# VinAIResearch/LFM

Measured on AMD Instinct MI355X. Metric: images/sec, higher is better.
Workload: dtype f16; 1 GPU; DiT-L/2 celeb256 f8 (4x32x32 latents), batch 64/GPU, 50-step Euler (torchdiffeq grid) + f8 VAE decode to 256x256 + uint8 NHWC; 2 batches in flight on 2 HIP streams (same weights, own scratch); per_gpu_batch=64, global_batch=64, h2d_of_latents=inside the timed step, nfe=50, batches_in_flight=2

## Files before the change

### include/lfm_hip.h

```cpp
#ifndef LFM_HIP_H
#define LFM_HIP_H
#include <stddef.h>
#include <stdint.h>

#ifdef __cplusplus
extern "C" {
#endif

typedef void* lfm_stream_t;

#define LFM_OK 0
#define LFM_ERR_SHAPE (-1)
#define LFM_ERR_ALIGN (-2)
#define LFM_ERR_WORKSPACE (-3)
#define LFM_ERR_LAUNCH (-4)
#define LFM_ERR_ARG (-5)

const char* lfm_strerror(int code);
#define LFM_ABI_VERSION 4
int lfm_abi_version(void);

typedef struct lfm_dit_shape {
  int depth;
  int hidden;
// ... 47 lines not shown
  int fold_ln;
  int gemm_select;
} lfm_dit_call;
#define LFM_CALL_OFF 1
#define LFM_CALL_ON 2
#define LFM_CALL_GEMM_SELECT(which) ((which) + 1)

size_t lfm_dit_workspace_bytes(const lfm_dit_shape* shape, int max_batch);

int lfm_dit_forward(const lfm_dit_shape* shape, const lfm_dit_weights* w, void* workspace, size_t workspace_bytes,
                    const lfm_dit_call* call, lfm_stream_t stream);

#define LFM_PLAN_FOLDED_LN 1
#define LFM_PLAN_FUSED_QKV_ATTENTION 2
int lfm_dit_plan(const lfm_dit_shape* shape, const lfm_dit_call* call, int* plan_out);

size_t lfm_dit_cond_table_bytes(const lfm_dit_shape* shape, int n_times);
int lfm_dit_cond_table_build(const lfm_dit_shape* shape, const lfm_dit_weights* w, void* workspace, size_t workspace_bytes, int batch, const float* t_values,
                             int n_times, void* table, size_t table_bytes, lfm_stream_t stream);

int lfm_gemm_f16(const void* A, long lda, const void* W, long ldw, void* C, long ldc, int M, int N, int K, const float* bias,
                 int epilogue, const float* gate, long gate_stride, int tokens, lfm_stream_t stream);

int lfm_gemm_qkv_f16(const void* A, long lda, const void* W, long ldw, void* Q, void* K_out, void* Vt, int M, int D, int K,
                     const float* bias, int head_dim, int tokens, lfm_stream_t stream);

int lfm_gemm_select(int which);
int lfm_gemm_plan(int M, int N, int K, int batch, int caps);

int lfm_profile_fc1(int enable);
int lfm_profile_blocks_read(float* host_ms_out, int max_n);
#define LFM_OPT_FOLD_LN 1
#define LFM_OPT_GEMM_V6 2
#define LFM_OPT_SKINNY_GEMM 4
#define LFM_OPT_ATTENTION_STREAM 5
#define LFM_OPT_FUSED_QKV_ATTENTION 6
int lfm_set_option(int key, int value);
int lfm_dit_call_settings(const lfm_dit_call* call, int* gemm_select_out, int* fold_ln_out);

int lfm_clock_probe(int blocks, int iters, unsigned long long* ticks_out, lfm_stream_t stream);

#ifdef LFM_MEASURE
int lfm_gemm_trace_read(unsigned long long* host_out, int n_per_group);
int lfm_attention_trace_read(unsigned long long* host_out, int n);
int lfm_attention_wg_trace_read(unsigned long long* host_out, int n_wg);
int lfm_dit_chk_arm(const void* workspace);
int lfm_dit_chk_read(unsigned long long* host_out, int n);
#endif
int lfm_profile_fc1_read(float* host_ms_out, int max_n);

int lfm_ln_modulate(const float* X, void* A, int M, int D, int tokens, const float* shift, const float* scale, long mod_stride,
// ... 95 lines not shown
```

### lfm_amd/csrc/dit.hip

```cpp
#include <mutex>

#include "../../include/lfm_hip.h"
#include "gemm_dispatch.h"
#include "gemm_skinny_kernel.h"
#include "gemm_sq64_kernel.h"
#include "qkv_attention_kernel.h"

typedef std::atomic<int> Opt;
static inline int opt_get(const Opt& o) { return o.load(std::memory_order_relaxed); }
static inline void opt_set(Opt& o, int v) { o.store(v, std::memory_order_relaxed); }
static struct {
  Opt gemm_sel{0}, gemm_dbg{0};
  Opt fold_ln{1};
  Opt v6{0};
  Opt skinny{1};
  Opt stagger{0};
  Opt att_stream{1};
  Opt fused_qkv{1};
} g_def;
static thread_local int tl_sel_set = 0, tl_gemm_sel = 0, tl_gemm_dbg = 0;
static thread_local int tl_fold = 0;
static inline int gemm_sel() { return tl_sel_set ? tl_gemm_sel : opt_get(g_def.gemm_sel); }
static inline int gemm_dbg() { return tl_sel_set ? tl_gemm_dbg : opt_get(g_def.gemm_dbg); }
static inline int opt_fold_ln() { return tl_fold ? (tl_fold == LFM_CALL_ON ? 1 : 0) : opt_get(g_def.fold_ln); }
int lfm_gemm_selected() { return gemm_sel(); }
int lfm_gemm_debug_flags() { return gemm_dbg(); }
int lfm_gemm_selected_v1_ok() { return gemm_sel() < 2 && !(gemm_dbg() & LFM_DBG_GEMM_NO_SPLITK); }
int lfm_gemm_prefers_v4(int M, int N, int K) {
  (void)M;
  (void)N;
  (void)K;
  if (gemm_dbg() & LFM_DBG_GEMM_NEVER_V4) return 0;
  if (gemm_dbg() & LFM_DBG_GEMM_ALWAYS_V4) return 1;
// ... 46 lines not shown
  }
  if (key == 2) {
    opt_set(g_def.v6, value != 0);
    return LFM_OK;
  }
  if (key == 4) {
    opt_set(g_def.skinny, value < 0 || value > 2 ? 1 : value);
    return LFM_OK;
  }
  if (key == 5) {
    opt_set(g_def.att_stream, value != 0);
    return LFM_OK;
  }
  if (key == 6) {
    opt_set(g_def.fused_qkv, value != 0);
    return LFM_OK;
  }
#ifdef LFM_MEASURE
  if (key == 3) {
    opt_set(g_def.stagger, value > 0 ? value : 0);
    return LFM_OK;
  }
#endif
  return LFM_ERR_ARG;
}
extern "C" int lfm_gemm_select(int which) {
  if (!gemm_select_valid(which)) return LFM_ERR_ARG;
  opt_set(g_def.gemm_sel, which & 15);
  opt_set(g_def.gemm_dbg, which >> 4);
  return LFM_OK;
// ... 1104 lines not shown
  const DitWs ws = carve(s, batch, workspace);
  if (ws.total > workspace_bytes) return LFM_ERR_WORKSPACE;
  if (((uintptr_t)workspace & 255) || ((uintptr_t)table & 15)) return LFM_ERR_ALIGN;
  hipStream_t st = (hipStream_t)stream;
  for (int i = 0; i < n_times; ++i) {
    rc = dit_conditioning(s, w, ws, t_values + i, 1, nullptr, 1, cond_uv_shape(s), st);
    if (rc) return rc;
    rc = dit_cond_copy(s, ws, (const float*)table, nullptr, 0, i, 1, st, n_times);
    if (rc) return rc;
  }
  return LFM_OK;
}

struct DitPlan {
  bool fold, w6, fused;
};
static DitPlan dit_plan(const lfm_dit_shape* s, int B, int rows) {
  const int D = s->hidden, H = s->mlp_hidden, grid = s->res / s->patch, T = grid * grid, M = B * T;
  const int tiles_p = D / 256;
  DitPlan p;
  p.fold = opt_fold_ln() && (D % 256 == 0) && (M % 256 == 0) && (rows == 1 || T % 256 == 0) && (long)(M / 256) * tiles_p >= 192 &&
           (gemm_sel() == 0 || gemm_sel() == 6) && (H % 64 == 0) && s->depth >= 1;
  p.w6 = gemm_sel() == 6 || (gemm_sel() == 0 && opt_get(g_def.v6));
  p.fused = p.fold && opt_get(g_def.fused_qkv) && !p.w6 && T == 256 && D == s->heads * 64 && (long)M * D < (1L << 31) && (long)3 * D * D < (1L << 31);
  return p;
}
extern "C" int lfm_dit_plan(const lfm_dit_shape* s, const lfm_dit_call* c, int* plan_out) {
  int rc = check_shape(s);
  if (rc) return rc;
  if (!c || !plan_out) return LFM_ERR_ARG;
  const int B = c->batch;
  if (B <= 0 || (c->t_len != 1 && c->t_len != B)) return LFM_ERR_SHAPE;
  CallScope scope;
  if ((rc = call_scope_enter(c)) != LFM_OK) return rc;
  const DitPlan p = dit_plan(s, B, (c->t_len == 1 && !c->y) ? 1 : B);
  *plan_out = (p.fold ? LFM_PLAN_FOLDED_LN : 0) | (p.fused ? LFM_PLAN_FUSED_QKV_ATTENTION : 0);
  return LFM_OK;
}

extern "C" int lfm_dit_forward(const lfm_dit_shape* s, const lfm_dit_weights* w, void* workspace, size_t workspace_bytes,
                               const lfm_dit_call* c, lfm_stream_t stream) {
  int rc = check_shape(s);
  if (rc) return rc;
  if (!w || !workspace || !c || !c->x || !c->t || !c->out) return LFM_ERR_ARG;
  const int B = c->batch;
  if (B <= 0 || (c->t_len != 1 && c->t_len != B)) return LFM_ERR_SHAPE;
  const bool cfg = c->cfg != 0;
  if (cfg && (B & 1)) return LFM_ERR_SHAPE;
  if (c->axpy_base && !c->axpy_dt) return LFM_ERR_ARG;
  const DitWs ws = carve(s, B, workspace);
  if (ws.total > workspace_bytes) return LFM_ERR_WORKSPACE;
// ... 47 lines not shown
  int cen_cur = 0;
  if (fold) {
    if (!pe_mfma) {
      hipLaunchKernelGGL(ln_center_mod_kernel, dim3(cdiv(M, 4)), dim3(256), 0, st, ws.X, ws.A, M, D, T, ws.mod + D, mstride, ws.ln_part, tiles_p,
                         ws.cen[0]);
      LFM_CHECK_LAUNCH();
    }
  }
  auto rowstat_src = [&]() {
    RowStatSrc r{ws.ln_part, ws.cen[cen_cur], ws.cen[cen_cur ^ 1], tiles_p, 1.0f / (float)D, 1e-6f};
    cen_cur ^= 1;
    return r;
  };
  auto launch_fold = [&](const ASrcRowMajor& a, const half_t* Wp, long ldw_, int M_, int N_, int K_, const auto& e) {
    return w6 ? launch_gemm256w_tn(a, Wp, ldw_, M_, N_, K_, e, st) : launch_gemm256h_tn(a, Wp, ldw_, M_, N_, K_, e, st);
  };
#ifdef LFM_MEASURE
  const bool chk = g_chk && workspace == g_chk_ws;
  if (chk) (void)hipMemsetAsync(g_chk, 0, DIT_CHK_SLOTS * 8, st);
#define DIT_CHK(buf, bytes, slot) \
  if (chk) dit_chk(buf, bytes, i, slot, st)
#else
#define DIT_CHK(buf, bytes, slot)
#endif
  const bool prof_blk = prof_ok && g_prof_blk_count < LFM_PROF_BLK_MAX;
  if (prof_blk) (void)hipEventRecord(g_prof_blk_ev[2 * g_prof_blk_count], st);
  const bool fused = plan.fused;
  if (fold) {
    for (int i = 0; i < s->depth; ++i) {
      const float* mod = ws.mod + (long)i * 6 * D;
// ... 3 lines not shown
      half_t* A1b = fused ? ws.A : ws.A2;
      if (fused) {
        const QkvAttnArgs e_qa{uq, uq + (long)rows * 3 * D, uvs_q, rowstat_src(), Ob, D, s->heads, 0.125f * 1.4426950408889634f, nullptr, 0};
        rc = launch_qkv_attention(ws.A, D, (const half_t*)w->qkv_w + (size_t)i * 3 * D * D, D, M, D, s->heads, D, e_qa, st);
        if (rc) return rc;
      } else {
        const EpiQKVMod e_qkv{Qb, Kb, Vb, uq, uq + (long)rows * 3 * D, uvs_q, D, D / s->heads, T, EpiQKV::log2_or_neg(T), rowstat_src(), nullptr, 0};
        rc = launch_fold(ASrcRowMajor{ws.A, D, M, 0}, (const half_t*)w->qkv_w + (size_t)i * 3 * D * D, D, M, 3 * D, D, e_qkv);
        if (rc) return rc;
        DIT_CHK(ws.QKVH, (size_t)3 * M * D * 2, 0);
        rc = attention_launch(Qb, Kb, Vb, Ob, B, s->heads, D / s->heads, T, st);
        if (rc) return rc;
      }
      DIT_CHK(Ob, (size_t)M * D * 2, 1);
      const EpiGateResidMod e_proj{ws.X, D, w->proj_b + (size_t)i * D, mod + 2 * D, mstride, T, A1b, mod + 4 * D, mstride, ws.cen[cen_cur], ws.ln_part, tiles_p};
      rc = launch_fold(ASrcRowMajor{Ob, D, M, 0}, (const half_t*)w->proj_w + (size_t)i * D * D, D, M, D, D, e_proj);
      if (rc) return rc;
      DIT_CHK(ws.X, (size_t)M * D * 4, 2);
      DIT_CHK(A1b, (size_t)M * D * 2, 3);
      DIT_CHK(ws.ln_part, (size_t)M * tiles_p * 8, 4);
      const bool prof = prof_ok && g_prof_mode == 1 && g_prof_count < LFM_PROF_MAX;
      if (prof) (void)hipEventRecord(g_prof_ev[2 * g_prof_count], st);
#if defined(LFM_MEASURE) && defined(LFM_EXP_DUMP)
      const EpiModGeluF16 e_fc1{ws.QKVH, H, uf, uf + (long)rows * H, uvs_f, T, rowstat_src(), nullptr, 0,
                                (g_dbg && workspace == g_dbg_ws) ? g_dbg + (long)i * g_dbg_stride : (float*)nullptr};
#else
      const EpiModGeluF16 e_fc1{ws.QKVH, H, uf, uf + (long)rows * H, uvs_f, T, rowstat_src(), nullptr, 0};
#endif
      rc = launch_fold(ASrcRowMajor{A1b, D, M, 0}, (const half_t*)w->fc1_w + (size_t)i * H * D, D, M, H, D, e_fc1);
      if (rc) return rc;
      if (prof) (void)hipEventRecord(g_prof_ev[2 * g_prof_count++ + 1], st);
      DIT_CHK(ws.QKVH, (size_t)M * H * 2, 5);
      if (i + 1 < s->depth) {
        const EpiGateResidMod e_fc2{ws.X, D, w->fc2_b + (size_t)i * D, mod + 5 * D, mstride, T, ws.A, mod + 7 * D, mstride, ws.cen[cen_cur], ws.ln_part, tiles_p};
        rc = launch_fold(ASrcRowMajor{ws.QKVH, H, M, 0}, (const half_t*)w->fc2_w + (size_t)i * D * H, H, M, D, H, e_fc2);
      } else {
        const EpiGateResidF32 e_fc2{ws.X, D, w->fc2_b + (size_t)i * D, mod + 5 * D, mstride, T};
        rc = launch_fold(ASrcRowMajor{ws.QKVH, H, M, 0}, (const half_t*)w->fc2_w + (size_t)i * D * H, H, M, D, H, e_fc2);
      }
      if (rc) return rc;
      DIT_CHK(ws.X, (size_t)M * D * 4, 6);
      DIT_CHK(ws.A, (size_t)M * D * 2, 7);
    }
  }
#undef DIT_CHK
  auto sk_slices = [&](int N_, int K_) {
    int sl = 1;
    while ((N_ / SK_BN) * (sl * 2) <= 256 && (K_ % (sl * 2 * SK_BK)) == 0 && K_ / (sl * 2) >= 2 * SK_BK && (size_t)(sl * 2) * M * N_ * 4 <= ws.slab_bytes) sl *= 2;
    return sl;
  };
// ... 170 lines not shown
```

### lfm_amd/csrc/gemm256h_kernel.h

```cpp
#pragma once
#include "gemm256n_kernel.h"

typedef float f32x4_t __attribute__((ext_vector_type(4)));

template <bool TRACE>
__device__ __forceinline__ void g256h_stamp(bool tr, int g, int wn, int lane, int slot) {
  if constexpr (TRACE) {
    if (tr && wn == 0 && lane == 0) {
      unsigned long long t;
      asm volatile("s_memtime %0\n\ts_waitcnt lgkmcnt(0)" : "=s"(t)::"memory");
      g256q_trace[g][slot] = t;
    }
  }
}

template <class Epi, class = void>
struct epi_has_row_aux {
  static constexpr bool value = false;
};
template <class Epi>
struct epi_has_row_aux<Epi, decltype((void)&Epi::row_aux)> {
  static constexpr bool value = true;
};

// ... 125 lines not shown
      for (int ps = 0; ps < 8; ++ps)
        if (mb + ps * 4 < M) epi.store(mb + ps * 4, n, v[ps], epi.load(mb + ps * 4, n));
    }
    asm volatile("s_waitcnt lgkmcnt(0)" ::: "memory");
  }
}

__device__ __forceinline__ float g256h_row16_sum(float v) {
  v = dpp_add<0xB1>(v);
  v = dpp_add<0x4E>(v);
  v = dpp_add<0x124>(v);
  v = dpp_add<0x128>(v);
  return v;
}

template <class Epi>
__device__ __forceinline__ void g256h_epilogue_mod(f32x4_t (&acc)[8][4], char* smem, const Epi& epi, int m0, int n0, int tile_n, int N, int g, int wn,
                                                   int lane, int wave) {
  char* scr = smem + wave * (32 * 272);
  float* red = (float*)(smem + 8 * 32 * 272);
  float* cen_s = (float*)(smem + 8 * 32 * 272 + 8192);
  const int l15 = lane & 15, l4 = lane >> 4;
  const int rrow = lane >> 4, rcol = lane & 15;
  const int n = n0 + wn * 64 + rcol * 4;
  const int img = m0 / epi.tokens;
  if (threadIdx.x < 256) cen_s[threadIdx.x] = epi.cen[m0 + threadIdx.x];
  const f32x4 bias = *(const f32x4*)(epi.bias + n);
  const f32x4 gate = *(const f32x4*)(epi.gate + (long)img * epi.gate_stride + n);
  const f32x4 sc1 = *(const f32x4*)(epi.scale + (long)img * epi.mod_stride + n) + 1.0f;
  __syncthreads();
#pragma unroll
  for (int i = 0; i < 4; ++i) {
#pragma unroll
    for (int h2 = 0; h2 < 2; ++h2)
#pragma unroll
      for (int j = 0; j < 4; ++j) *(f32x4_t*)(scr + (h2 * 16 + l15) * 272 + (j * 16 + l4 * 4) * 4) = acc[2 * i + h2][j];
    asm volatile("s_waitcnt lgkmcnt(0)" ::: "memory");
    const int rl = g * 128 + i * 32 + rrow;
    f32x4 xo[8];
#pragma unroll
    for (int ps = 0; ps < 8; ++ps) xo[ps] = *(const f32x4*)(epi.X + (long)(m0 + rl + ps * 4) * epi.ldx + n);
#pragma unroll
    for (int ps = 0; ps < 8; ++ps) {
      const f32x4 v = *(const f32x4*)(scr + (ps * 4 + rrow) * 272 + rcol * 16);
      const float c = cen_s[rl + ps * 4];
      const f32x4 xn = xo[ps] + gate * (v + bias);
      *(f32x4*)(epi.X + (long)(m0 + rl + ps * 4) * epi.ldx + n) = xn;
      const f32x4 d = xn - c;
      const f32x4 ap = d * sc1;
      const half4_t h = {(half_t)ap.x, (half_t)ap.y, (half_t)ap.z, (half_t)ap.w};
      *(half4_t*)(epi.A + (long)(m0 + rl + ps * 4) * N + n) = h;
      const float sx = g256h_row16_sum((xn.x + xn.y) + (xn.z + xn.w));
      const float sq = g256h_row16_sum((d.x * d.x + d.y * d.y) + (d.z * d.z + d.w * d.w));
      if (rcol == 0) {
        float* dst = red + (((g * 4 + wn) * 128) + i * 32 + ps * 4 + rrow) * 2;
        dst[0] = sx;
// ... 6 lines not shown
  if (wn == 0) {
#pragma unroll
    for (int rr = 0; rr < 2; ++rr) {
      const int r = lane + 64 * rr;
      float sx = 0.f, sq = 0.f;
#pragma unroll
      for (int w4 = 0; w4 < 4; ++w4) {
        sx += red[((g * 4 + w4) * 128 + r) * 2];
        sq += red[((g * 4 + w4) * 128 + r) * 2 + 1];
      }
      *(f32x2*)(epi.part + ((long)(m0 + g * 128 + r) * epi.tiles_n + tile_n) * 2) = (f32x2){sx, sq};
    }
  }
}

#define G256H_MAX_PARTS 5
struct G256hRowStatRegs {
  f32x2 p[G256H_MAX_PARTS];
  float c;
};
template <class Epi>
__device__ __forceinline__ G256hRowStatRegs g256h_rowstat_load(const Epi& epi, int m0, int M) {
  G256hRowStatRegs r;
  const int m = m0 + (int)threadIdx.x < M ? m0 + (int)threadIdx.x : M - 1;
  if (threadIdx.x < 256) {
    const f32x2* pp = (const f32x2*)(epi.st.part + (long)m * epi.st.tiles_p * 2);
#pragma unroll
    for (int t = 0; t < G256H_MAX_PARTS; ++t) r.p[t] = t < epi.st.tiles_p ? pp[t] : (f32x2){0.f, 0.f};
    r.c = epi.st.cen_in[m];
  }
// ... 163 lines not shown

  typename ASrc::Row arow[2][2];
  const half_t* wrow[2][2];
  const int cswz = ((tid & 7) ^ ((tid >> 4) & 7)) * 8;
#pragma unroll
  for (int s = 0; s < 2; ++s)
#pragma unroll
    for (int p = 0; p < 2; ++p) {
      arow[s][p] = asrc.row(m0 + p * 128 + s * 64 + (tid >> 3));
      const int n = n0 + (p * 2 + (tid >> 8)) * 64 + s * 32 + ((tid >> 3) & 31);
      wrow[s][p] = W + (long)(n < N ? n : N - 1) * ldw + cswz;
    }
  const int nk = K / G256Q_BK;
  const int dma_off = wave * 1024;
  bool dma_on = true;
  constexpr bool BUFDMA = (OPT & 1) != 0 && asrc_has_buffer<ASrc>::value;
  __amdgpu_buffer_rsrc_t rsa, rsw;
  unsigned avoff[2][2], wvoff[2][2];
  if constexpr (BUFDMA) {
    rsa = asrc.rsrc();
    rsw = __builtin_amdgcn_make_buffer_rsrc((void*)W, 0, -1, 0x00020000);
#pragma unroll
    for (int s = 0; s < 2; ++s)
#pragma unroll
      for (int p = 0; p < 2; ++p) {
        avoff[s][p] = asrc.voff(arow[s][p], cswz);
        const int n = n0 + (p * 2 + (tid >> 8)) * 64 + s * 32 + ((tid >> 3) & 31);
        wvoff[s][p] = ((unsigned)(n < N ? n : N - 1) * (unsigned)ldw + (unsigned)cswz) * 2u;
      }
  }
// ... 59 lines not shown
        }
        return;
      }
      if constexpr (PH == 0) {
        if (s1) issue_b(1, t + 1, oth + G256Q_SLOT_B1, P);
      } else if constexpr (PH == 1) {
        if (s1) issue_a(1, oth + G256Q_SLOT_A1, P);
      } else if constexpr (PH == 2) {
        if (s2) {
          if (P != 2) asrc.begin_tile(t + 2, G256Q_BK);
          issue_a(0, cur + G256Q_SLOT_A0, P);
        }
      } else {
        if (s2) issue_b(0, t + 2, cur + G256Q_SLOT_B0, P);
      }
    };
    if constexpr ((OPT & 2) != 0) {
      stage(1);
      __builtin_amdgcn_sched_barrier(0);
    }
    if constexpr (PH == 0) {
#pragma unroll
      for (int ks = 0; ks < 2; ++ks) {
        lds_read(wf[0][ks], w_addr[ks] + HI, g256q_ic<G256Q_SLOT_B0>{});
        lds_read(wf[1][ks], w_addr[ks] + HI, g256q_ic<G256Q_SLOT_B0 + 2048>{});
        lds_read(af[0][ks], a_addr[ks] + HI, g256q_ic<G256Q_SLOT_A0>{});
        lds_read(af[1][ks], a_addr[ks] + HI, g256q_ic<G256Q_SLOT_A0 + 2048>{});
        lds_read(af[2][ks], a_addr[ks] + HI, g256q_ic<G256Q_SLOT_A0 + 4096>{});
        lds_read(af[3][ks], a_addr[ks] + HI, g256q_ic<G256Q_SLOT_A0 + 6144>{});
      }
// ... 2 lines not shown
      for (int ks = 0; ks < 2; ++ks) {
        lds_read(wf[2][ks], w_addr[ks] + HI, g256q_ic<G256Q_SLOT_B1>{});
        lds_read(wf[3][ks], w_addr[ks] + HI, g256q_ic<G256Q_SLOT_B1 + 2048>{});
      }
    } else if constexpr (PH == 2) {
#pragma unroll
      for (int ks = 0; ks < 2; ++ks) {
        lds_read(af[0][ks], a_addr[ks] + HI, g256q_ic<G256Q_SLOT_A1>{});
        lds_read(af[1][ks], a_addr[ks] + HI, g256q_ic<G256Q_SLOT_A1 + 2048>{});
        lds_read(af[2][ks], a_addr[ks] + HI, g256q_ic<G256Q_SLOT_A1 + 4096>{});
        lds_read(af[3][ks], a_addr[ks] + HI, g256q_ic<G256Q_SLOT_A1 + 6144>{});
      }
    }
    __builtin_amdgcn_sched_barrier(0);
    stage((OPT & 2) != 0 ? 2 : 0);
    if constexpr (ABL == 1 || ABL == 3 || (ABL >= 5 && ABL <= 7)) {
      G256H_VMCNT(0);
    } else if constexpr ((OPT & 4) != 0) {
      if (s1) {
        if constexpr (PH < 3) G256H_VMCNT(4);
        else if (s2) G256H_VMCNT(6);
        else G256H_VMCNT(2);
      } else G256H_VMCNT(0);
    } else if (s2) G256H_VMCNT(6);
    else if (s1) {
      if constexpr (PH < 2) G256H_VMCNT(6);
      else if constexpr (PH == 2) G256H_VMCNT(4);
      else G256H_VMCNT(2);
    } else G256H_VMCNT(0);
  };
  auto mfma_part = [&](auto PHC, auto SWC) {
// ... 42 lines not shown
            if constexpr (SW) asm volatile("v_mfma_f32_16x16x32_f16 %0, %1, %2, %0" : "+v"(acc[I0 + i4][J0 + j2]) : "v"(af[i4][ks]), "v"(wf[J0 + j2][ks]));
            else asm volatile("v_mfma_f32_16x16x32_f16 %0, %1, %2, %0" : "+v"(acc[I0 + i4][J0 + j2]) : "v"(wf[J0 + j2][ks]), "v"(af[i4][ks]));
          } else if constexpr (SW) acc[I0 + i4][J0 + j2] = __builtin_amdgcn_mfma_f32_16x16x32_f16(af[i4][ks], wf[J0 + j2][ks], acc[I0 + i4][J0 + j2], 0, 0, 0);
          else acc[I0 + i4][J0 + j2] = __builtin_amdgcn_mfma_f32_16x16x32_f16(wf[J0 + j2][ks], af[i4][ks], acc[I0 + i4][J0 + j2], 0, 0, 0);
        }
        __builtin_amdgcn_sched_barrier(0);
      }
    if constexpr (ABL != 4) __builtin_amdgcn_s_setprio(0);
  };

  G256hRowStatRegs rsr;
  if constexpr (epi_has_rowstat<Epi>::value) {
    rsr = g256h_rowstat_load(epi, m0, M);
    __builtin_amdgcn_sched_barrier(0);
  }
  asrc.begin_tile(0, G256Q_BK);
  issue_a(0, smem + G256Q_SLOT_A0);
  issue_b(0, 0, smem + G256Q_SLOT_B0);
  issue_b(1, 0, smem + G256Q_SLOT_B1);
  issue_a(1, smem + G256Q_SLOT_A1);
  if (nk > 1) {
    asrc.begin_tile(1, G256Q_BK);
    issue_a(0, smem + G256Q_BUF_BYTES + G256Q_SLOT_A0);
    issue_b(0, 1, smem + G256Q_BUF_BYTES + G256Q_SLOT_B0);
  }
  if constexpr (epi_has_rowstat<Epi>::value) g256h_rowstat_finish(epi, rsr, smem, m0, M, tile_n);
  if (nk > 1) G256H_VMCNT(6);
  else G256H_VMCNT(2);
  if constexpr (ABL == 1 || ABL == 3 || (ABL >= 5 && ABL <= 7)) {
    G256H_VMCNT(0);
    dma_on = false;
  }
  if constexpr (ABL == 2 || ABL == 3 || (ABL >= 5 && ABL <= 7)) {
#pragma unroll
    for (int i = 0; i < 4; ++i)
#pragma unroll
      for (int ks = 0; ks < 2; ++ks) {
        af[i][ks] = (half8_t){1, 2, 3, 4, 5, 6, 7, 8};
        wf[i][ks] = (half8_t){1, -1, 1, -1, 1, -1, 1, -1};
      }
  }
  if constexpr (ABL == 4) {
    if (g == 1) __builtin_amdgcn_s_setprio(1);
  }
  G256_BARRIER();
  auto run = [&](auto GC, auto SWC) {
    constexpr int G = decltype(GC)::value;
    if constexpr (G == 0) load_part(g256q_ic<0>{}, g256q_ic<0>{}, 0, 1 < nk, 2 < nk);
    G256_BARRIER();
    auto tile = [&](auto BUFC, int t) {
      constexpr int BUF = decltype(BUFC)::value;
      const bool s1 = t + 1 < nk, s2 = t + 2 < nk, s3 = t + 3 < nk;
      auto phase = [&](auto PHC) {
        constexpr int PH = decltype(PHC)::value;
        if constexpr (G == 0) {
          mfma_part(PHC, SWC);
          if constexpr (PH < 3) load_part(g256q_ic<PH + 1>{}, BUFC, t, s1, s2);
          else if (s1) load_part(g256q_ic<0>{}, g256q_ic<(BUF ^ 1)>{}, t + 1, s2, s3);
        } else {
          load_part(PHC, BUFC, t, s1, s2);
          mfma_part(PHC, SWC);
        }
        if constexpr (ABL == 5 || ABL == 7) {
        } else if constexpr (ABL == 6) {
// ... 17 lines not shown
  if constexpr (epi_has_transposed<Epi>::value) {
    if (swapped) {
      if (g == 0) run(g256q_ic<0>{}, g256q_ic<1>{});
      else run(g256q_ic<1>{}, g256q_ic<1>{});
    } else {
      if (g == 0) run(g256q_ic<0>{}, g256q_ic<0>{});
      else run(g256q_ic<1>{}, g256q_ic<0>{});
    }
  } else {
    if (g == 0) run(g256q_ic<0>{}, g256q_ic<0>{});
    else run(g256q_ic<1>{}, g256q_ic<0>{});
  }
#undef G256H_VMCNT
#undef G256H_LGKM
  if constexpr (ABL == 7 || ABL == 8) asm volatile("s_nop 7\n\ts_nop 7\n\ts_nop 7" ::: "memory");
  g256h_epilogue<G256_BN, TRACE>(acc, smem, epi, m0, n0, M, N, g, wn, lane, wave, bz, bsC, dbg, swapped);
}

template <class ASrc, class Epi, bool TRACE = false, int ABL = 0, int OPT = G256H_DEFAULT_OPT>
static inline int launch_gemm256h_tn(const ASrc& asrc, const half_t* W, long ldw, int M, int N, int K, const Epi& epi, hipStream_t stream,
                                     int batch = 1, long bsA = 0, long bsW = 0, long bsC = 0) {
  if (!asrc_fits(asrc, 0)) return LFM_ERR_SHAPE;
  if constexpr ((OPT & 1) != 0 && asrc_has_buffer<ASrc>::value) {
    if (!asrc_fits_buffer(asrc, 0) || (long)N * ldw >= (1L << 31)) return LFM_ERR_SHAPE;
  }
  if (M <= 0 || N <= 0 || K <= 0 || (K % G256Q_BK) != 0 || (N % 4) != 0) return LFM_ERR_SHAPE;
  if ((ldw % 8) != 0 || ((uintptr_t)W & 15)) return LFM_ERR_ALIGN;
  const int tm = cdiv(M, G256_BM), tn = cdiv(N, G256_BN);
  constexpr int LDS = G256Q_LDS_BYTES + (epi_has_rowstat<Epi>::value ? 2048 : 0);
  static lfm_device_mask attr_set{0};
  const unsigned long long dbit = lfm_device_bit();
  if (lfm_device_todo(attr_set, dbit)) {
    if (hipFuncSetAttribute((const void*)gemm256h_tn_kernel<ASrc, Epi, TRACE, ABL, OPT>, hipFuncAttributeMaxDynamicSharedMemorySize, LDS) != hipSuccess)
      return LFM_ERR_LAUNCH;
    lfm_device_done(attr_set, dbit);
  }
  hipLaunchKernelGGL((gemm256h_tn_kernel<ASrc, Epi, TRACE, ABL, OPT>), dim3(tm * tn, batch), dim3(512), LDS, stream, asrc, W, ldw, M, N, K, tn, epi, bsA,
                     bsW, bsC, lfm_gemm_debug_flags());
  LFM_CHECK_LAUNCH();
  return LFM_OK;
}
```

### lfm_amd/csrc/gemm_kernel.h

```cpp
#pragma once
#include "common.h"
#include "debug_flags.h"

#define GEMM_BM 128
#define GEMM_BN 128
#define GEMM_BK 64
#define GEMM_STAGE_BYTES (2 * GEMM_BM * GEMM_BK * 2)
#define GEMM_LDS_BYTES (2 * GEMM_STAGE_BYTES)

struct ASrcRowMajor {
  const half_t* A;
  long lda;
  int M;
  __device__ __forceinline__ void init(int bz, long bs) { A += (long)bz * bs; }
  struct Row {
    unsigned off;
  };
  __device__ __forceinline__ Row row(int m) const {
    Row r;
    r.off = (unsigned)((m < M ? m : M - 1) * (int)lda);
    return r;
  }
  int k0;
  __device__ __forceinline__ void begin_tile(int kt, int bk) { k0 = kt * bk; }
// ... 164 lines not shown
    a.x = *(const f32x4*)(X + (long)m * ldx + n);
    return a;
  }
  __device__ __forceinline__ void store(int m, int n, f32x4 v, const Aux& a) const {
    *(f32x4*)(X + (long)m * ldx + n) = a.x + a.g * (v + a.b);
  }
};
template <class Epi, class = void>
struct epi_is_producer_mod {
  static constexpr bool value = false;
};
template <class Epi>
struct epi_is_producer_mod<Epi, decltype((void)Epi::producer_mod)> {
  static constexpr bool value = Epi::producer_mod;
};

struct EpiModF16 {
  half_t* C;
  long ldc;
  const float* u;
  const float* v;
  long uv_stride;
  int tokens;
  const float* rs;
  int m0;
  struct Aux {
    f32x4 u, v;
  };
  static constexpr bool column_aux = true;
  __device__ __forceinline__ Aux load(int m, int n) const {
// ... 569 lines not shown
```

### lfm_amd/hip.py

```python
import ctypes as C
import os

import torch

_HERE = os.path.dirname(os.path.abspath(__file__))
LIB_PATH = os.path.join(_HERE, "_lib", "liblfm_hip.so")
_lib = None


class LfmHipError(RuntimeError):
    pass


class DitShape(C.Structure):
    _fields_ = [(n, C.c_int) for n in ("depth", "hidden", "heads", "patch", "in_ch", "res", "mlp_hidden", "label_rows")]


_DIT_WEIGHT_FIELDS = ("pos_embed", "patch_w", "patch_b", "t_w0", "t_b0", "t_w2", "t_b2", "y_table", "ada_w", "ada_b",
                      "qkv_w", "qkv_b", "proj_w", "proj_b", "fc1_w", "fc1_b", "fc2_w", "fc2_b", "final_w", "final_b", "patch_w16")


class DitWeights(C.Structure):
    _fields_ = [(n, C.c_void_p) for n in _DIT_WEIGHT_FIELDS]

# ... 69 lines not shown
    L.lfm_profile_fc1.argtypes = [C.c_int]
    L.lfm_profile_fc1_read.restype = C.c_int
    L.lfm_profile_fc1_read.argtypes = [C.POINTER(C.c_float), C.c_int]
    L.lfm_profile_blocks_read.restype = C.c_int
    L.lfm_profile_blocks_read.argtypes = [C.POINTER(C.c_float), C.c_int]
    L.lfm_ln_modulate.restype = C.c_int
    L.lfm_ln_modulate.argtypes = [C.c_void_p, C.c_void_p, C.c_int, C.c_int, C.c_int, C.c_void_p, C.c_void_p, C.c_long, C.c_void_p]
    L.lfm_dit_attention.restype = C.c_int
    L.lfm_dit_attention.argtypes = [C.c_void_p, C.c_void_p, C.c_void_p, C.c_void_p, C.c_int, C.c_int, C.c_int, C.c_void_p]
    L.lfm_set_option.restype = C.c_int
    L.lfm_set_option.argtypes = [C.c_int, C.c_int]
    L.lfm_dit_call_settings.restype = C.c_int
    L.lfm_dit_call_settings.argtypes = [C.POINTER(DitCall), C.POINTER(C.c_int), C.POINTER(C.c_int)]
    L.lfm_dit_plan.restype = C.c_int
    L.lfm_dit_plan.argtypes = [C.POINTER(DitShape), C.POINTER(DitCall), C.POINTER(C.c_int)]
    L.lfm_gemm_plan.restype = C.c_int
    L.lfm_gemm_plan.argtypes = [C.c_int] * 5
    L.lfm_dit_attention_hd.restype = C.c_int
    L.lfm_dit_attention_hd.argtypes = [C.c_void_p, C.c_void_p, C.c_void_p, C.c_void_p, C.c_int, C.c_int, C.c_int, C.c_int, C.c_void_p]
    L.lfm_grid_advance.restype = C.c_int
    L.lfm_grid_advance.argtypes = [C.c_void_p] * 7
    L.lfm_lincomb.restype = C.c_int
    L.lfm_lincomb.argtypes = [C.c_void_p, C.c_void_p, C.POINTER(C.c_void_p), C.c_void_p, C.c_void_p, C.c_int, C.c_long, C.c_void_p]
    L.lfm_rk_error_norm.restype = C.c_int
    L.lfm_rk_error_norm.argtypes = [C.c_void_p, C.c_void_p, C.POINTER(C.c_void_p), C.c_void_p, C.c_void_p, C.c_int, C.c_long, C.c_float, C.c_float,
                                    C.c_void_p, C.c_void_p, C.c_void_p]
    L.lfm_vae_workspace_bytes.restype = C.c_size_t
    L.lfm_vae_workspace_bytes.argtypes = [C.c_int, C.c_int]
    L.lfm_vae_decode.restype = C.c_int
    L.lfm_vae_decode.argtypes = [C.c_void_p, C.c_void_p, C.c_size_t, C.c_void_p, C.c_void_p, C.c_int, C.c_int, C.c_int, C.c_void_p]
# ... 149 lines not shown
DBG_LN_FOUR_ROWS = 262144
DBG_LN_TWO_ROWS = 524288
DBG_DIT_FINAL_ROUND1 = 1048576
DBG_DIT_PATCH_ROUND1 = 2097152
DBG_CONV_IMPLICIT_GEMM = 8388608
DBG_CONV_HALO_SMALL = 16777216
DBG_VAE_SEPARATE_STATS = 4194304
DBG_UNET_CONV_IN_SCALAR = 1
DBG_UNET_ATT_VALU = 16
DBG_UNET_GN_ROWS = 16384

OPT_FOLD_LN = 1
OPT_SKINNY_GEMM = 4
OPT_ATTENTION_STREAM = 5
OPT_FUSED_QKV_ATTENTION = 6
OPT_GEMM_V6 = 2


def effective_clock_mhz(device=None, iters=20000):
    dev = torch.device(device or "cuda:0")
    n = torch.cuda.get_device_properties(dev).multi_processor_count
    ticks = torch.zeros(n, dtype=torch.int64, device=dev)
    for it in (200, iters):
        e0, e1 = torch.cuda.Event(enable_timing=True), torch.cuda.Event(enable_timing=True)
        e0.record(torch.cuda.current_stream(dev))
        check(lib().lfm_clock_probe(n, it, ptr(ticks), stream_ptr(dev)), "lfm_clock_probe")
        e1.record(torch.cuda.current_stream(dev))
        torch.cuda.synchronize(dev)
    ms = e0.elapsed_time(e1)
    return 2.0 * float(ticks.max()) / (ms * 1e3)


PLAN_FOLDED_LN, PLAN_FUSED_QKV_ATTENTION = 1, 2


def dit_plan(shape, batch, t_len=1, labels=False, fold_ln=0, gemm_select=0):
    call = DitCall()
    call.batch, call.t_len, call.y = int(batch), int(t_len), (1 if labels else None)
    call.fold_ln, call.gemm_select = fold_ln, gemm_select
    plan = C.c_int(-1)
    check(lib().lfm_dit_plan(C.byref(shape), C.byref(call), C.byref(plan)), "lfm_dit_plan")
    return plan.value


GEMM_CAP_V6, GEMM_CAP_FITS = 1, 2


def gemm_plan(M, N, K, batch=1, caps=GEMM_CAP_V6 | GEMM_CAP_FITS):
    return lib().lfm_gemm_plan(int(M), int(N), int(K), int(batch), int(caps))


def set_option(key, value):
    check(lib().lfm_set_option(int(key), int(value)), "lfm_set_option")


def vt_token_perm(T, device=None):
    i = torch.arange(T, device=device)
    return (i & ~12) | ((i & 4) << 1) | ((i & 8) >> 1)

# ... 22 lines not shown
```

Baseline: 121.4 images/sec.

## Prefetch residual X and epilogue constants into LDS during producer GEMM main loop

Adds a prefetching variant of the proj and fc2 producer GEMM epilogue. Part of the fp32 residual X tile is copied into LDS with buffer-to-LDS DMA in otherwise idle slots of the last K-tiles, and the per-tile cen, bias, gate and scale values are loaded up front and parked in LDS. The aim is to hide the epilogue's global-memory latency behind the MFMA loop. In exchange it uses more LDS per workgroup, which may lower occupancy, adds a separate main-loop path with hand-tuned vmcnt waits, and is on by default behind a new option.

```diff
diff --git a/include/lfm_hip.h b/include/lfm_hip.h
--- a/include/lfm_hip.h
+++ b/include/lfm_hip.h
@@ -85,6 +85,7 @@
 #define LFM_PLAN_FOLDED_LN 1
 #define LFM_PLAN_FUSED_QKV_ATTENTION 2
 int lfm_dit_plan(const lfm_dit_shape* shape, const lfm_dit_call* call, int* plan_out);
+int lfm_dit_producer_prefetch(const lfm_dit_shape* shape, const lfm_dit_call* call, int* on_out);
 
 size_t lfm_dit_cond_table_bytes(const lfm_dit_shape* shape, int n_times);
 int lfm_dit_cond_table_build(const lfm_dit_shape* shape, const lfm_dit_weights* w, void* workspace, size_t workspace_bytes, int batch, const float* t_values,
@@ -106,6 +107,7 @@
 #define LFM_OPT_SKINNY_GEMM 4
 #define LFM_OPT_ATTENTION_STREAM 5
 #define LFM_OPT_FUSED_QKV_ATTENTION 6
+#define LFM_OPT_PRODUCER_PREFETCH 7
 int lfm_set_option(int key, int value);
 int lfm_dit_call_settings(const lfm_dit_call* call, int* gemm_select_out, int* fold_ln_out);
 
diff --git a/lfm_amd/csrc/dit.hip b/lfm_amd/csrc/dit.hip
--- a/lfm_amd/csrc/dit.hip
+++ b/lfm_amd/csrc/dit.hip
@@ -17,6 +17,7 @@
   Opt stagger{0};
   Opt att_stream{1};
   Opt fused_qkv{1};
+  Opt prod_pf{1};
 } g_def;
 static thread_local int tl_sel_set = 0, tl_gemm_sel = 0, tl_gemm_dbg = 0;
 static thread_local int tl_fold = 0;
@@ -93,6 +94,10 @@
   }
   if (key == 6) {
     opt_set(g_def.fused_qkv, value != 0);
+    return LFM_OK;
+  }
+  if (key == 7) {
+    opt_set(g_def.prod_pf, value != 0);
     return LFM_OK;
   }
 #ifdef LFM_MEASURE
@@ -1227,6 +1232,7 @@
 
 struct DitPlan {
   bool fold, w6, fused;
+  bool prod_pf;
 };
 static DitPlan dit_plan(const lfm_dit_shape* s, int B, int rows) {
   const int D = s->hidden, H = s->mlp_hidden, grid = s->res / s->patch, T = grid * grid, M = B * T;
@@ -1236,6 +1242,7 @@
            (gemm_sel() == 0 || gemm_sel() == 6) && (H % 64 == 0) && s->depth >= 1;
   p.w6 = gemm_sel() == 6 || (gemm_sel() == 0 && opt_get(g_def.v6));
   p.fused = p.fold && opt_get(g_def.fused_qkv) && !p.w6 && T == 256 && D == s->heads * 64 && (long)M * D < (1L << 31) && (long)3 * D * D < (1L << 31);
+  p.prod_pf = p.fold && opt_get(g_def.prod_pf) && !p.w6 && (H % 128) == 0 && (long)M * D < (1L << 30);
   return p;
 }
 extern "C" int lfm_dit_plan(const lfm_dit_shape* s, const lfm_dit_call* c, int* plan_out) {
@@ -1248,6 +1255,17 @@
   if ((rc = call_scope_enter(c)) != LFM_OK) return rc;
   const DitPlan p = dit_plan(s, B, (c->t_len == 1 && !c->y) ? 1 : B);
   *plan_out = (p.fold ? LFM_PLAN_FOLDED_LN : 0) | (p.fused ? LFM_PLAN_FUSED_QKV_ATTENTION : 0);
+  return LFM_OK;
+}
+extern "C" int lfm_dit_producer_prefetch(const lfm_dit_shape* s, const lfm_dit_call* c, int* on_out) {
+  int rc = check_shape(s);
+  if (rc) return rc;
+  if (!c || !on_out) return LFM_ERR_ARG;
+  const int B = c->batch;
+  if (B <= 0 || (c->t_len != 1 && c->t_len != B)) return LFM_ERR_SHAPE;
+  CallScope scope;
+  if ((rc = call_scope_enter(c)) != LFM_OK) return rc;
+  *on_out = dit_plan(s, B, (c->t_len == 1 && !c->y) ? 1 : B).prod_pf ? 1 : 0;
   return LFM_OK;
 }
 
@@ -1325,6 +1343,10 @@
   };
   auto launch_fold = [&](const ASrcRowMajor& a, const half_t* Wp, long ldw_, int M_, int N_, int K_, const auto& e) {
     return w6 ? launch_gemm256w_tn(a, Wp, ldw_, M_, N_, K_, e, st) : launch_gemm256h_tn(a, Wp, ldw_, M_, N_, K_, e, st);
+  };
+  const bool prod_pf = plan.prod_pf;
+  auto launch_producer = [&](const ASrcRowMajor& a, const half_t* Wp, long ldw_, int M_, int N_, int K_, const EpiGateResidMod& e) {
+    return prod_pf ? launch_gemm256h_tn(a, Wp, ldw_, M_, N_, K_, EpiGateResidModPF{e}, st) : launch_fold(a, Wp, ldw_, M_, N_, K_, e);
   };
 #ifdef LFM_MEASURE
   const bool chk = g_chk && workspace == g_chk_ws;
@@ -1358,7 +1380,7 @@
       }
       DIT_CHK(Ob, (size_t)M * D * 2, 1);
       const EpiGateResidMod e_proj{ws.X, D, w->proj_b + (size_t)i * D, mod + 2 * D, mstride, T, A1b, mod + 4 * D, mstride, ws.cen[cen_cur], ws.ln_part, tiles_p};
-      rc = launch_fold(ASrcRowMajor{Ob, D, M, 0}, (const half_t*)w->proj_w + (size_t)i * D * D, D, M, D, D, e_proj);
+      rc = launch_producer(ASrcRowMajor{Ob, D, M, 0}, (const half_t*)w->proj_w + (size_t)i * D * D, D, M, D, D, e_proj);
       if (rc) return rc;
       DIT_CHK(ws.X, (size_t)M * D * 4, 2);
       DIT_CHK(A1b, (size_t)M * D * 2, 3);
@@ -1377,7 +1399,7 @@
       DIT_CHK(ws.QKVH, (size_t)M * H * 2, 5);
       if (i + 1 < s->depth) {
         const EpiGateResidMod e_fc2{ws.X, D, w->fc2_b + (size_t)i * D, mod + 5 * D, mstride, T, ws.A, mod + 7 * D, mstride, ws.cen[cen_cur], ws.ln_part, tiles_p};
-        rc = launch_fold(ASrcRowMajor{ws.QKVH, H, M, 0}, (const half_t*)w->fc2_w + (size_t)i * D * H, H, M, D, H, e_fc2);
+        rc = launch_producer(ASrcRowMajor{ws.QKVH, H, M, 0}, (const half_t*)w->fc2_w + (size_t)i * D * H, H, M, D, H, e_fc2);
       } else {
         const EpiGateResidF32 e_fc2{ws.X, D, w->fc2_b + (size_t)i * D, mod + 5 * D, mstride, T};
         rc = launch_fold(ASrcRowMajor{ws.QKVH, H, M, 0}, (const half_t*)w->fc2_w + (size_t)i * D * H, H, M, D, H, e_fc2);
diff --git a/lfm_amd/csrc/gemm256h_kernel.h b/lfm_amd/csrc/gemm256h_kernel.h
--- a/lfm_amd/csrc/gemm256h_kernel.h
+++ b/lfm_amd/csrc/gemm256h_kernel.h
@@ -163,21 +163,36 @@
   return v;
 }
 
-template <class Epi>
+#define G256H_PROD_SCR (G256Q_BUF_BYTES)
+#define G256H_PROD_CONST (G256H_PROD_SCR + 8 * 32 * 272 + 8192)
+#define G256H_PROD_LDS_BYTES (G256H_PROD_CONST + 4096)
+template <class Epi, bool PF = false>
 __device__ __forceinline__ void g256h_epilogue_mod(f32x4_t (&acc)[8][4], char* smem, const Epi& epi, int m0, int n0, int tile_n, int N, int g, int wn,
                                                    int lane, int wave) {
+  char* const xlds = smem + wave * 1024 + lane * 16;
+  if constexpr (PF) smem += G256H_PROD_SCR;
   char* scr = smem + wave * (32 * 272);
   float* red = (float*)(smem + 8 * 32 * 272);
   float* cen_s = (float*)(smem + 8 * 32 * 272 + 8192);
   const int l15 = lane & 15, l4 = lane >> 4;
   const int rrow = lane >> 4, rcol = lane & 15;
   const int n = n0 + wn * 64 + rcol * 4;
-  const int img = m0 / epi.tokens;
-  if (threadIdx.x < 256) cen_s[threadIdx.x] = epi.cen[m0 + threadIdx.x];
-  const f32x4 bias = *(const f32x4*)(epi.bias + n);
-  const f32x4 gate = *(const f32x4*)(epi.gate + (long)img * epi.gate_stride + n);
-  const f32x4 sc1 = *(const f32x4*)(epi.scale + (long)img * epi.mod_stride + n) + 1.0f;
-  __syncthreads();
+  f32x4 bias, gate, sc1;
+  if constexpr (PF) {
+    const float* cs = cen_s + 256 + wn * 64 + rcol * 4;
+    bias = *(const f32x4*)cs;
+    gate = *(const f32x4*)(cs + 256);
+    sc1 = *(const f32x4*)(cs + 512) + 1.0f;
+    asm volatile("s_waitcnt vmcnt(0)" ::: "memory");
+    G256_BARRIER();
+  } else {
+    const int img = m0 / epi.tokens;
+    if (threadIdx.x < 256) cen_s[threadIdx.x] = epi.cen[m0 + threadIdx.x];
+    bias = *(const f32x4*)(epi.bias + n);
+    gate = *(const f32x4*)(epi.gate + (long)img * epi.gate_stride + n);
+    sc1 = *(const f32x4*)(epi.scale + (long)img * epi.mod_stride + n) + 1.0f;
+    __syncthreads();
+  }
 #pragma unroll
   for (int i = 0; i < 4; ++i) {
 #pragma unroll
@@ -188,7 +203,10 @@
     const int rl = g * 128 + i * 32 + rrow;
     f32x4 xo[8];
 #pragma unroll
-    for (int ps = 0; ps < 8; ++ps) xo[ps] = *(const f32x4*)(epi.X + (long)(m0 + rl + ps * 4) * epi.ldx + n);
+    for (int ps = 0; ps < 8; ++ps) {
+      if (PF && i == 1) xo[ps] = *(const f32x4*)(xlds + ps * 8192);
+      else xo[ps] = *(const f32x4*)(epi.X + (long)(m0 + rl + ps * 4) * epi.ldx + n);
+    }
 #pragma unroll
     for (int ps = 0; ps < 8; ++ps) {
       const f32x4 v = *(const f32x4*)(scr + (ps * 4 + rrow) * 272 + rcol * 16);
@@ -225,6 +243,50 @@
   }
 }
 
+struct G256hProdConst {
+  float cen, bias, gate, scale;
+};
+template <class Epi>
+__device__ __forceinline__ G256hProdConst g256h_prod_const_load(const Epi& epi, int m0, int n0) {
+  G256hProdConst r{};
+  if (threadIdx.x < 256) {
+    const long img = m0 / epi.tokens;
+    r.cen = epi.cen[m0 + threadIdx.x];
+    r.bias = epi.bias[n0 + threadIdx.x];
+    r.gate = epi.gate[img * epi.gate_stride + n0 + threadIdx.x];
+    r.scale = epi.scale[img * epi.mod_stride + n0 + threadIdx.x];
+  }
+  return r;
+}
+__device__ __forceinline__ void g256h_prod_const_park(const G256hProdConst& r, char* smem) {
+  float* cs = (float*)(smem + G256H_PROD_CONST);
+  if (threadIdx.x < 256) {
+    cs[threadIdx.x] = r.cen;
+    cs[256 + threadIdx.x] = r.bias;
+    cs[512 + threadIdx.x] = r.gate;
+    cs[768 + threadIdx.x] = r.scale;
+  }
+}
+template <class Epi>
+__device__ __forceinline__ __amdgpu_buffer_rsrc_t g256h_prod_x_rsrc(const Epi& epi) {
+  return __builtin_amdgcn_make_buffer_rsrc((void*)epi.X, 0, -1, 0x00020000);
+}
+template <class Epi>
+__device__ __forceinline__ unsigned g256h_prod_x_voff(const Epi& epi, int m0, int n0, int g, int wn, int lane) {
+  return ((unsigned)(m0 + g * 128 + (lane >> 4)) * (unsigned)epi.ldx + (unsigned)(n0 + wn * 64 + (lane & 15) * 4)) * 4u;
+}
+template <class Epi>
+__device__ __forceinline__ unsigned g256h_prod_x_soff(const Epi& epi, int ps) {
+  return (unsigned)(32 + ps * 4) * (unsigned)epi.ldx * 4u;
+}
+template <class Epi>
+__device__ __forceinline__ void g256h_prod_x_dma(int ps, char* slot_wave, const Epi& epi, int m0, int n0, int g, int wn, int lane) {
+  const __amdgpu_buffer_rsrc_t rx = g256h_prod_x_rsrc(epi);
+  const unsigned vo = g256h_prod_x_voff(epi, m0, n0, g, wn, lane);
+  glds16_buf(rx, vo, g256h_prod_x_soff(epi, ps), slot_wave);
+  glds16_buf(rx, vo, g256h_prod_x_soff(epi, ps + 1), slot_wave + 8192);
+}
+
 #define G256H_MAX_PARTS 5
 struct G256hRowStatRegs {
   f32x2 p[G256H_MAX_PARTS];
@@ -418,6 +480,8 @@
   const int nk = K / G256Q_BK;
   const int dma_off = wave * 1024;
   bool dma_on = true;
+  constexpr bool PFX = epi_prefetch_x<Epi>::value;
+  static_assert(!PFX || (ABL == 0 && (OPT & 6) == 0), "the prefetching epilogue counts on the default DMA placement");
   constexpr bool BUFDMA = (OPT & 1) != 0 && asrc_has_buffer<ASrc>::value;
   __amdgpu_buffer_rsrc_t rsa, rsw;
   unsigned avoff[2][2], wvoff[2][2];
@@ -507,6 +571,17 @@
       } else {
         if (s2) issue_b(0, t + 2, cur + G256Q_SLOT_B0, P);
       }
+      if constexpr (PFX) {
+        if constexpr (PH == 2) {
+          if (s1 && !s2) g256h_prod_x_dma(0, cur + G256Q_SLOT_A0 + dma_off, epi, m0, n0, g, wn, lane);
+        } else if constexpr (PH == 3) {
+          if (s1 && !s2) g256h_prod_x_dma(2, cur + G256Q_SLOT_B0 + dma_off, epi, m0, n0, g, wn, lane);
+        } else if constexpr (PH == 0) {
+          if (!s1) g256h_prod_x_dma(4, oth + G256Q_SLOT_B1 + dma_off, epi, m0, n0, g, wn, lane);
+        } else {
+          if (!s1) g256h_prod_x_dma(6, oth + G256Q_SLOT_A1 + dma_off, epi, m0, n0, g, wn, lane);
+        }
+      }
     };
     if constexpr ((OPT & 2) != 0) {
       stage(1);
@@ -539,7 +614,11 @@
     }
     __builtin_amdgcn_sched_barrier(0);
     stage((OPT & 2) != 0 ? 2 : 0);
-    if constexpr (ABL == 1 || ABL == 3 || (ABL >= 5 && ABL <= 7)) {
+    if constexpr (PFX) {
+      if (s1) G256H_VMCNT(6);
+      else if constexpr (PH == 0) G256H_VMCNT(6);
+      else G256H_VMCNT(8);
+    } else if constexpr (ABL == 1 || ABL == 3 || (ABL >= 5 && ABL <= 7)) {
       G256H_VMCNT(0);
     } else if constexpr ((OPT & 4) != 0) {
       if (s1) {
@@ -612,6 +691,11 @@
     rsr = g256h_rowstat_load(epi, m0, M);
     __builtin_amdgcn_sched_barrier(0);
   }
+  G256hProdConst pcr;
+  if constexpr (PFX) {
+    pcr = g256h_prod_const_load(epi, m0, n0);
+    __builtin_amdgcn_sched_barrier(0);
+  }
   asrc.begin_tile(0, G256Q_BK);
   issue_a(0, smem + G256Q_SLOT_A0);
   issue_b(0, 0, smem + G256Q_SLOT_B0);
@@ -623,6 +707,7 @@
     issue_b(0, 1, smem + G256Q_BUF_BYTES + G256Q_SLOT_B0);
   }
   if constexpr (epi_has_rowstat<Epi>::value) g256h_rowstat_finish(epi, rsr, smem, m0, M, tile_n);
+  if constexpr (PFX) g256h_prod_const_park(pcr, smem);
   if (nk > 1) G256H_VMCNT(6);
   else G256H_VMCNT(2);
   if constexpr (ABL == 1 || ABL == 3 || (ABL >= 5 && ABL <= 7)) {
@@ -646,6 +731,35 @@
     constexpr int G = decltype(GC)::value;
     if constexpr (G == 0) load_part(g256q_ic<0>{}, g256q_ic<0>{}, 0, 1 < nk, 2 < nk);
     G256_BARRIER();
+    if constexpr (PFX) {
+      auto tile_pf = [&](auto BUFC, int t, bool s1, bool s2, bool s3) __attribute__((always_inline)) {
+        constexpr int BUF = decltype(BUFC)::value;
+        auto phase = [&](auto PHC) {
+          constexpr int PH = decltype(PHC)::value;
+          if constexpr (G == 0) {
+            mfma_part(PHC, SWC);
+            if constexpr (PH < 3) load_part(g256q_ic<PH + 1>{}, BUFC, t, s1, s2);
+            else if (s1) load_part(g256q_ic<0>{}, g256q_ic<(BUF ^ 1)>{}, t + 1, s2, s3);
+          } else {
+            load_part(PHC, BUFC, t, s1, s2);
+            mfma_part(PHC, SWC);
+          }
+          G256_BARRIER();
+        };
+        phase(g256q_ic<0>{});
+        phase(g256q_ic<1>{});
+        phase(g256q_ic<2>{});
+        phase(g256q_ic<3>{});
+      };
+      int t = 0;
+      for (; t + 3 < nk; t += 2) {
+        tile_pf(g256q_ic<0>{}, t, true, true, true);
+        tile_pf(g256q_ic<1>{}, t + 1, true, true, t + 4 < nk);
+      }
+      tile_pf(g256q_ic<0>{}, t, true, false, false);
+      tile_pf(g256q_ic<1>{}, t + 1, false, false, false);
+      return;
+    }
     auto tile = [&](auto BUFC, int t) {
       constexpr int BUF = decltype(BUFC)::value;
       const bool s1 = t + 1 < nk, s2 = t + 2 < nk, s3 = t + 3 < nk;
@@ -693,7 +807,11 @@
 #undef G256H_VMCNT
 #undef G256H_LGKM
   if constexpr (ABL == 7 || ABL == 8) asm volatile("s_nop 7\n\ts_nop 7\n\ts_nop 7" ::: "memory");
-  g256h_epilogue<G256_BN, TRACE>(acc, smem, epi, m0, n0, M, N, g, wn, lane, wave, bz, bsC, dbg, swapped);
+  if constexpr (PFX) {
+    if (!(dbg & LFM_DBG_GEMM_NO_EPILOGUE)) g256h_epilogue_mod<Epi, true>(acc, smem, epi, m0, n0, n0 / G256_BN, N, g, wn, lane, wave);
+  } else {
+    g256h_epilogue<G256_BN, TRACE>(acc, smem, epi, m0, n0, M, N, g, wn, lane, wave, bz, bsC, dbg, swapped);
+  }
 }
 
 template <class ASrc, class Epi, bool TRACE = false, int ABL = 0, int OPT = G256H_DEFAULT_OPT>
@@ -704,9 +822,13 @@
     if (!asrc_fits_buffer(asrc, 0) || (long)N * ldw >= (1L << 31)) return LFM_ERR_SHAPE;
   }
   if (M <= 0 || N <= 0 || K <= 0 || (K % G256Q_BK) != 0 || (N % 4) != 0) return LFM_ERR_SHAPE;
+  if constexpr (epi_prefetch_x<Epi>::value) {
+    if ((K % (2 * G256Q_BK)) != 0 || epi.ldx <= 0 || (long)M * epi.ldx * 4 >= (1L << 32)) return LFM_ERR_SHAPE;
+  }
   if ((ldw % 8) != 0 || ((uintptr_t)W & 15)) return LFM_ERR_ALIGN;
   const int tm = cdiv(M, G256_BM), tn = cdiv(N, G256_BN);
-  constexpr int LDS = G256Q_LDS_BYTES + (epi_has_rowstat<Epi>::value ? 2048 : 0);
+  constexpr int LDS = epi_prefetch_x<Epi>::value ? G256H_PROD_LDS_BYTES
+                                                      : G256Q_LDS_BYTES + (epi_has_rowstat<Epi>::value ? 2048 : 0);
   static lfm_device_mask attr_set{0};
   const unsigned long long dbit = lfm_device_bit();
   if (lfm_device_todo(attr_set, dbit)) {
diff --git a/lfm_amd/csrc/gemm_kernel.h b/lfm_amd/csrc/gemm_kernel.h
--- a/lfm_amd/csrc/gemm_kernel.h
+++ b/lfm_amd/csrc/gemm_kernel.h
@@ -202,6 +202,17 @@
 struct epi_is_producer_mod<Epi, decltype((void)Epi::producer_mod)> {
   static constexpr bool value = Epi::producer_mod;
 };
+struct EpiGateResidModPF : EpiGateResidMod {
+  static constexpr bool prefetch_x = true;
+};
+template <class Epi, class = void>
+struct epi_prefetch_x {
+  static constexpr bool value = false;
+};
+template <class Epi>
+struct epi_prefetch_x<Epi, decltype((void)Epi::prefetch_x)> {
+  static constexpr bool value = Epi::prefetch_x;
+};
 
 struct EpiModF16 {
   half_t* C;
diff --git a/lfm_amd/hip.py b/lfm_amd/hip.py
--- a/lfm_amd/hip.py
+++ b/lfm_amd/hip.py
@@ -107,6 +107,8 @@
     L.lfm_dit_call_settings.argtypes = [C.POINTER(DitCall), C.POINTER(C.c_int), C.POINTER(C.c_int)]
     L.lfm_dit_plan.restype = C.c_int
     L.lfm_dit_plan.argtypes = [C.POINTER(DitShape), C.POINTER(DitCall), C.POINTER(C.c_int)]
+    L.lfm_dit_producer_prefetch.restype = C.c_int
+    L.lfm_dit_producer_prefetch.argtypes = [C.POINTER(DitShape), C.POINTER(DitCall), C.POINTER(C.c_int)]
     L.lfm_gemm_plan.restype = C.c_int
     L.lfm_gemm_plan.argtypes = [C.c_int] * 5
     L.lfm_dit_attention_hd.restype = C.c_int
@@ -286,6 +288,7 @@
 OPT_SKINNY_GEMM = 4
 OPT_ATTENTION_STREAM = 5
 OPT_FUSED_QKV_ATTENTION = 6
+OPT_PRODUCER_PREFETCH = 7
 OPT_GEMM_V6 = 2
 
 
@@ -315,6 +318,15 @@
     return plan.value
 
 
+def dit_producer_prefetch(shape, batch, t_len=1, labels=False, fold_ln=0, gemm_select=0):
+    call = DitCall()
+    call.batch, call.t_len, call.y = int(batch), int(t_len), (1 if labels else None)
+    call.fold_ln, call.gemm_select = fold_ln, gemm_select
+    on = C.c_int(-1)
+    check(lib().lfm_dit_producer_prefetch(C.byref(shape), C.byref(call), C.byref(on)), "lfm_dit_producer_prefetch")
+    return on.value
+
+
 GEMM_CAP_V6, GEMM_CAP_FITS = 1, 2
 
 
```

After: 122.6 images/sec, median of 6. No clear change (+1.0%).
